# aleksandrina-streltsova/lidar-global-registration

Measured on AMD Instinct MI355X. Metric: scan-pair registrations/sec, higher is better.
Workload: dtype f32

## Files before the change

### lidar-global-registration_amd/csrc/lgr_match_sweep.cuh

```cuda
#pragma once
#include "lgr_match_common.cuh"
#include "lgr_match_mfma.cuh"

namespace {

constexpr int SW_RB = 1;
constexpr int SW_OCC = SW_RB == 1 ? 6 : 4;

__global__ void ucol_pack_kernel(const float* __restrict__ u_colv, int mb_pad, float c_scale, unsigned short* __restrict__ out) {
    const int col = blockIdx.x * blockDim.x + threadIdx.x;
    if (col >= mb_pad) return;
    const float t = ((fmaxf(u_colv[col], 0.f) * 1.00001f) * 1.0001f) * c_scale;
    const unsigned bits = t >= 0.f ? __float_as_uint(t) : 0x7f800000u;
    out[col] = (unsigned short) (min(bits + 0xffffu, 0x7f800000u) >> 16);
}

__global__ void pass_select_kernel(const unsigned long long* __restrict__ pass_stages, double half_of_all, const int* __restrict__ xcd_start ,
                                   int* __restrict__ xs_sweep, int* __restrict__ xs_plain) {
    const int i = threadIdx.x;
    if (i >= 9) return;
    const bool plain = pass_stages && (double) pass_stages[0] > half_of_all;
    xs_sweep[i] = plain ? 0 : xcd_start[i];
    xs_plain[i] = plain ? xcd_start[i] : 0;
}

__global__ __launch_bounds__(NTHR, SW_OCC) void match_sweep(const f16x8* __restrict__ Ap, const f16x8* __restrict__ Bp, size_t bset_stride ,
                                                            float c_scale, const int* __restrict__ blkcl, int ma_pad, int mb_pad, int rg_rows,
                                                            const unsigned* __restrict__ stage_mask, int n_cc, int item_rb, const int2* __restrict__ items,
                                                            const int* __restrict__ xcd_start, int* __restrict__ xcd_ctr, CoarseArgs ca,
                                                            const unsigned short* __restrict__ ucol16 ,
                                                            uint2* __restrict__ kept_out, unsigned long long* __restrict__ kept_count , unsigned kept_cap) {
    typedef f16x8 frag;
    constexpr int NF = OpFmt<FMT_F16R>::NF;
    constexpr int STAGE_FRAGS = STAGE_TILES * NF * 64;
    constexpr int CO_FRAGS = STAGE_TILES * 2 * 64, CO_NB = 6, CO_D = 4;
    static_assert(CO_D == 4 && CO_NB == CO_D + 2, "the counted waits below are written for two pairs of stages in flight");
    static_assert(WAVES == 2 * STAGE_TILES, "one coarse piece per wave");
    __shared__ __attribute__((aligned(16))) unsigned char smem[CO_NB * CO_FRAGS * (int) sizeof(frag) + 16];
    int& item_s = *reinterpret_cast<int*>(smem + CO_NB * CO_FRAGS * (int) sizeof(frag));
    unsigned n_tested = 0u, n_rejected = 0u, n_skipped = 0u;
    const int xcd = blockIdx.x % 8;
    const int item0 = xcd_start[xcd], n_items = xcd_start[xcd + 1] - item0;
    const int tid = threadIdx.x, lane = tid & 63, wave = tid >> 6, half = lane >> 5;
    const int rg_blocks = rg_rows / BLOCK_ROWS;
    const int n_rb_total = ma_pad / BLOCK_ROWS;
    constexpr int IINF = 0x7f800000;
    const f32x16 nav = {0.f, 0.f, 0.f, 0.f, 0.f, 0.f, 0.f, 0.f, 0.f, 0.f, 0.f, 0.f, 0.f, 0.f, 0.f, 0.f};

    for (;;) {
        __syncthreads();
        if (tid == 0) item_s = n_items > 0 ? atomicAdd(&xcd_ctr[xcd], 1) : 0x7fffffff;
        __syncthreads();
        const int it = item_s;
        if (it >= n_items) break;
        const int2 item = items[item0 + it];
        const int cc = item.x, rb0 = item.y;
        const int n_rb = min(item_rb, n_rb_total - rb0);
        const int col_tile0 = cc * (CHUNK_COLS / TILE);
        const int n_coltiles = min(CHUNK_COLS / TILE, mb_pad / TILE - col_tile0);
        const int n_stages = n_coltiles / STAGE_TILES;
        const unsigned full = n_stages >= 32 ? 0xffffffffu : ((1u << n_stages) - 1u);
        unsigned my_mask = lane < n_rb ? (stage_mask[(size_t) (rb0 + lane) * n_cc + cc] & full) : 0u;

        for (int rbi = 0; rbi < n_rb;) {
            const int rbA = rb0 + rbi;
            const bool pair = SW_RB == 2 && rbi + 1 < n_rb && blkcl[rbA + 1] == blkcl[rbA];
            const unsigned mk[2] = {(unsigned) __builtin_amdgcn_readlane(my_mask, rbi), pair ? (unsigned) __builtin_amdgcn_readlane(my_mask, min(rbi + 1, 63)) : 0u};
            rbi += pair ? 2 : 1;
            const unsigned mask = mk[0] | mk[1];
            if (!mask) continue;
            const int set = blkcl[rbA];
            const frag* Bset = Bp + (size_t) set * bset_stride + (size_t) col_tile0 * NF * 64;
            int row_tile[2];
            frag a0[2], a1[2];
            int t_lane[2][2];
            float e_lane[2][2];
            float trow[2];
            unsigned long long skipm[2][2];
            unsigned kept[2][STAGE_TILES];
            const unsigned skipped_before = n_skipped;
#pragma unroll
            for (int r = 0; r < SW_RB; ++r) {
                row_tile[r] = (rbA + r) * (BLOCK_ROWS / TILE) + wave;
                const int rt = mk[r] ? row_tile[r] : row_tile[0];
                a0[r] = Ap[((size_t) rt * NF + 0) * 64 + lane];
                a1[r] = Ap[((size_t) rt * NF + 1) * 64 + lane];
                t_lane[r][0] = t_lane[r][1] = IINF; e_lane[r][0] = e_lane[r][1] = 0.f; trow[r] = 0.f;
                skipm[r][0] = skipm[r][1] = 0ull;
#pragma unroll
                for (int ct = 0; ct < STAGE_TILES; ++ct) kept[r][ct] = 0u;
            }
            asm volatile("s_waitcnt lgkmcnt(0)\n\ts_barrier" : : : "memory");
            unsigned to_issue = mask, to_do = mask;
            int issued = 0, done_ = 0;
            auto dma_coarse = [&]() {
                const int s_ = __builtin_ctz(to_issue);
                to_issue &= to_issue - 1u;
                const char* src = reinterpret_cast<const char*>(Bset + (size_t) s_ * STAGE_FRAGS + (size_t) ((wave >> 1) * NF + (wave & 1)) * 64);
                char* dst = reinterpret_cast<char*>(smem) + (issued % CO_NB) * (CO_FRAGS * (int) sizeof(frag)) + wave * 1024;
#ifndef LGR_EXP_SWEEP_NODMA
                __builtin_amdgcn_global_load_lds((const void*) (src + lane * 16), (__attribute__((address_space(3))) void*) dst, 16, 0, 0);
#else
                (void) src; (void) dst;
#endif
                ++issued;
            };
            while (issued < CO_D && to_issue) dma_coarse();
#pragma unroll
            for (int r = 0; r < SW_RB; ++r) {
                if (!mk[r]) continue;
                const int rb = rbA + r;
                const float ur = ca.u_rt[rb * (BLOCK_ROWS / TILE) + wave];
                if (ca.u_row) trow[r] = ((fmaxf(ca.u_row[(size_t) row_tile[r] * TILE + (lane & 31)], 0.f) * 1.00001f) * 1.0001f) * c_scale;
                const float x = ca.xmax[rb / rg_blocks];
#pragma unroll
                for (int h2 = 0; h2 < 2; ++h2) {
                    if (!(h2 ? (mk[r] >> 16) : (mk[r] & 0xffffu))) continue;
                    const int q = lane + 64 * h2;
                    const int gst = min(cc * STAGES_PER_CHUNK + (q >> 2), ca.n_stage_total - 1);
                    const int gct = min(col_tile0 + q, ca.n_ct_total - 1);
                    const float us = ca.u_stage ? __uint_as_float(ca.u_ct[gct]) : 0.f;
                    float xt = x, yt = ca.ymax[(size_t) set * ca.n_stage_total + gst];
                    if (ca.rt_shell) {
                        const float2 sa = ca.rt_shell[rb * (BLOCK_ROWS / TILE) + wave];
                        const float2 sb = ca.ct_shell[(size_t) set * ca.n_ct_total + gct];
                        const float gap = fmaxf(sb.x - sa.y, sa.x - sb.y) - 4e-6f * (sa.y + sb.y);
                        const float U = fmaxf(fmaxf(ur, us), 0.f);
                        const bool skip = gap > 0.f && gap * gap * (0.99999f * 0.99999f * 0.99999f) > U * 1.00001f + 1e-12f;
                        skipm[r][h2] = __ballot(skip);
                        xt = fminf(xt, sa.y); yt = fminf(yt, sb.y);
                    }
                    const float s = xt + yt;
                    const float et = (ca.quad * s) * s + ca.cross * (xt * yt) + ca.lin * s + ca.abs;
                    float t = fmaxf(fmaxf(ca.u_row ? 0.f : ur, us), 0.f) * 1.00001f + et;
                    t = (t * 1.0001f) * c_scale;
                    t_lane[r][h2] = t >= 0.f ? __float_as_int(t) : IINF;
                    e_lane[r][h2] = (et * 1.0001f) * c_scale;
                }
            }
            asm volatile("" : : "v"(t_lane[0][0]), "v"(t_lane[0][1]), "v"(e_lane[0][0]), "v"(e_lane[0][1]), "v"(trow[0]) : "memory");
            if (SW_RB == 2) asm volatile("" : : "v"(t_lane[1][0]), "v"(t_lane[1][1]), "v"(e_lane[1][0]), "v"(e_lane[1][1]), "v"(trow[1]) : "memory");
            auto compute = [&](int st, int buf) {
                const frag* cs = reinterpret_cast<const frag*>(smem) + buf * CO_FRAGS + lane;
                unsigned need[2];
#pragma unroll
                for (int r = 0; r < SW_RB; ++r) {
                    const unsigned sk4 = (unsigned) ((st < 16 ? skipm[r][0] : skipm[r][1]) >> ((st * STAGE_TILES) & 63)) & 0xfu;
                    const bool on = (mk[r] >> st) & 1u;
                    if (on) n_skipped += (unsigned) __builtin_popcount(sk4);
                    need[r] = on ? (~sk4 & 0xfu) : 0u;
                }
                if (!(need[0] | (SW_RB == 2 ? need[1] : 0u))) return;
#pragma unroll
                for (int ct = 0; ct < STAGE_TILES; ++ct) {
                    if (!(((need[0] | (SW_RB == 2 ? need[1] : 0u)) >> ct) & 1u)) continue;
                    const int q = st * STAGE_TILES + ct;
                    const frag c0 = cs[ct * 128], c1 = cs[ct * 128 + 64];
#pragma unroll
                    for (int r = 0; r < SW_RB; ++r) {
                        if (!((need[r] >> ct) & 1u)) continue;
                        f32x16 acc = mfma_step(c0, a0[r], nav);
                        acc = mfma_step(c1, a1[r], acc);
                        auto ai = [&](int g) { return __float_as_int(acc[g]); };
                        const int m0 = min(min(ai(0), ai(1)), ai(2)), m1 = min(min(ai(3), ai(4)), ai(5)), m2 = min(min(ai(6), ai(7)), ai(8));
                        const int m3 = min(min(ai(9), ai(10)), ai(11)), m4 = min(min(ai(12), ai(13)), ai(14));
                        const int m = min(min(min(m0, m1), m2), min(min(m3, m4), ai(15)));
                        const int t_sel = st < 16 ? t_lane[r][0] : t_lane[r][1];
                        const float e_sel = st < 16 ? e_lane[r][0] : e_lane[r][1];
                        const int tc = __builtin_amdgcn_readlane(t_sel, q & 63);
                        const float te = __uint_as_float(__builtin_amdgcn_readlane(__float_as_uint(e_sel), q & 63));
                        const int thr = max(__float_as_int(trow[r] + te), tc);
                        if (__ballot(m <= thr) == 0ull) continue;
                        bool kp = __ballot(m <= __float_as_int(trow[r] + te)) != 0ull;
                        if (!kp && ucol16) {
                            const unsigned short* uc = ucol16 + ((size_t) (col_tile0 + q) << 5) + 4 * half;
                            float dmin = 3.4028234663852886e38f;
#pragma unroll
                            for (int gq = 0; gq < 4; ++gq) {
                                const uint2 w = *reinterpret_cast<const uint2*>(uc + 8 * gq);
                                const float u0 = __uint_as_float(w.x << 16), u1 = __uint_as_float(w.x & 0xffff0000u);
                                const float u2 = __uint_as_float(w.y << 16), u3 = __uint_as_float(w.y & 0xffff0000u);
                                dmin = fminf(fminf(dmin, acc[4 * gq] - u0), acc[4 * gq + 1] - u1);
                                dmin = fminf(fminf(dmin, acc[4 * gq + 2] - u2), acc[4 * gq + 3] - u3);
                            }
                            kp = __ballot(dmin <= te) != 0ull;
                        } else if (!kp && !ucol16) kp = true;
                        if (kp) kept[r][ct] |= 1u << st;
                    }
                }
            };
            while (to_do) {
                const int st = __builtin_ctz(to_do);
                to_do &= to_do - 1u;
                int st2 = -1;
                if (to_do) { st2 = __builtin_ctz(to_do); to_do &= to_do - 1u; }
                const int n_now = st2 >= 0 ? 2 : 1;
                const int newer = issued - done_ - n_now;
                if (newer >= 2) asm volatile("s_waitcnt vmcnt(2)" : : : "memory");
                else if (newer == 1) asm volatile("s_waitcnt vmcnt(1)" : : : "memory");
                else asm volatile("s_waitcnt vmcnt(0)" : : : "memory");
                __builtin_amdgcn_s_barrier();
                if (to_issue) dma_coarse();
                if (to_issue) dma_coarse();
#ifndef LGR_EXP_SWEEP_NOCOMPUTE
                compute(st, done_ % CO_NB);
                if (st2 >= 0) compute(st2, (done_ + 1) % CO_NB);
#endif
                done_ += n_now;
            }
            unsigned nk = 0u;
#pragma unroll
            for (int r = 0; r < SW_RB; ++r)
#pragma unroll
                for (int ct = 0; ct < STAGE_TILES; ++ct) nk += (unsigned) __builtin_popcount(kept[r][ct]);
            {
                const unsigned swept = (unsigned) (STAGE_TILES * (__builtin_popcount(mk[0]) + (SW_RB == 2 ? __builtin_popcount(mk[1]) : 0))), sk_now = n_skipped - skipped_before;
                n_tested += swept - sk_now;
                n_rejected += swept - sk_now - nk;
            }
            if (nk) {
                unsigned long long base = 0ull;
                if (lane == 0) base = atomicAdd(kept_count, (unsigned long long) nk);
                base = ((unsigned long long) (unsigned) __builtin_amdgcn_readfirstlane((int) (base >> 32)) << 32) | (unsigned) __builtin_amdgcn_readfirstlane((int) (unsigned) base);
                unsigned off = 0u;
#pragma unroll
                for (int r = 0; r < SW_RB; ++r)
#pragma unroll
                    for (int ct = 0; ct < STAGE_TILES; ++ct) {
                        const unsigned m = kept[r][ct];
                        if (lane < 32 && ((m >> lane) & 1u)) {
                            const unsigned long long pos = base + off + (unsigned) __builtin_popcount(m & ((1u << lane) - 1u));
                            if (pos < (unsigned long long) kept_cap) kept_out[pos] = make_uint2((unsigned) row_tile[r], (unsigned) (col_tile0 + lane * STAGE_TILES + ct));
                        }
                        off += (unsigned) __builtin_popcount(m);
                    }
            }
        }
    }
    if (ca.cnt && lane == 0) {
        if (n_tested) atomicAdd(&ca.cnt[0], (unsigned long long) n_tested);
        if (n_rejected) atomicAdd(&ca.cnt[1], (unsigned long long) n_rejected);
        if (n_skipped) atomicAdd(&ca.cnt[2], (unsigned long long) n_skipped);
    }
}

__global__ void touched_kernel(const uint2* __restrict__ kept, const unsigned long long* __restrict__ kept_count, unsigned kept_cap, const int* __restrict__ xs_plain ,
                               const uint8_t* __restrict__ sched, const int* __restrict__ tile_leaf, int n_leaves, size_t n_pairs, uint8_t* __restrict__ touched ) {
    const size_t i0 = (size_t) blockIdx.x * blockDim.x + threadIdx.x, step = (size_t) gridDim.x * blockDim.x;
    if (xs_plain[8] > 0 || *kept_count > (unsigned long long) kept_cap) {
        for (size_t i = i0; i < n_pairs; i += step) touched[i] = sched[i];
        return;
    }
    const size_t n = (size_t) *kept_count;
    for (size_t e = i0; e < n; e += step) {
        const uint2 ent = kept[e];
        const size_t idx = (size_t) (ent.x / (BLOCK_ROWS / TILE)) * n_leaves + tile_leaf[ent.y];
        touched[idx] = sched[idx];
    }
}

constexpr int TL_WAVES = 4, TL_RUN = 4;
template <bool COLDIR>
__global__ __launch_bounds__(64 * TL_WAVES) void match_tiles(const f16x8* __restrict__ Ap, const f16x8* __restrict__ Bp, size_t bset_stride, float out_scale,
                                                             const int* __restrict__ blkcl, int ma_pad, int mb_pad, int rg_rows, const int* __restrict__ tile_group,
                                                             int* __restrict__ rowmin, int* __restrict__ colmin, const uint2* __restrict__ kept,
                                                             const unsigned long long* __restrict__ kept_count, unsigned kept_cap) {
    typedef f16x8 frag;
    constexpr int NF = OpFmt<FMT_F16R>::NF;
    constexpr int IINF = 0x7f800000;
    const int lane = threadIdx.x & 63, half = lane >> 5;
    if (*kept_count > (unsigned long long) kept_cap) return;
    const unsigned n = (unsigned) *kept_count;
    const unsigned n_waves = gridDim.x * TL_WAVES, w_id = blockIdx.x * TL_WAVES + (threadIdx.x >> 6);
    const int rg_blocks = rg_rows / BLOCK_ROWS;
    const f32x16 nav = {0.f, 0.f, 0.f, 0.f, 0.f, 0.f, 0.f, 0.f, 0.f, 0.f, 0.f, 0.f, 0.f, 0.f, 0.f, 0.f};
    frag a[NF];
    unsigned cur_rt = 0xffffffffu;
    for (unsigned e0 = w_id * TL_RUN; e0 < n; e0 += n_waves * TL_RUN) {
        for (unsigned e = e0; e < min(n, e0 + TL_RUN); ++e) {
            const uint2 ent = kept[e];
            const unsigned rt = ent.x, ct = ent.y;
            const int rb = (int) (rt / (BLOCK_ROWS / TILE));
            if (rt != cur_rt) {
                cur_rt = rt;
#pragma unroll
                for (int kk = 0; kk < NF; ++kk) a[kk] = Ap[((size_t) rt * NF + kk) * 64 + lane];
            }
            const frag* bsrc = Bp + (size_t) blkcl[rb] * bset_stride + (size_t) ct * NF * 64 + lane;
            frag b[NF];
#pragma unroll
            for (int kk = 0; kk < NF; ++kk) b[kk] = bsrc[kk * 64];
            const f32x16 acc = mfma_chain<FMT_F16R>(a, b, nav);
            if (COLDIR) {
                int cm = min(__float_as_int(acc[0]), __float_as_int(acc[1]));
#pragma unroll
                for (int g = 2; g < 16; g += 2) cm = min(min(cm, __float_as_int(acc[g])), __float_as_int(acc[g + 1]));
                cm = min(cm, __shfl_xor(cm, 32));
                if (lane < 32 && cm != IINF) {
                    const int v = __float_as_int(__int_as_float(cm) * out_scale);
                    atomicMin(&colmin[(size_t) (rb / rg_blocks) * mb_pad + (size_t) ct * TILE + lane], v);
                }
            }
            {
                int rmin[16];
#pragma unroll
                for (int g = 0; g < 16; ++g) rmin[g] = __float_as_int(acc[g]);
                int w8[8], w4[4], w2[2], w1;
#pragma unroll
                for (int j = 0; j < 8; ++j) {
                    auto sw = __builtin_amdgcn_permlane16_swap((unsigned) rmin[j], (unsigned) rmin[8 + j], false, false);
                    w8[j] = min((int) sw[0], (int) sw[1]);
                }
                {
                    const bool up = (lane & 8) != 0;
#pragma unroll
                    for (int j = 0; j < 4; ++j) {
                        int keep = up ? w8[4 + j] : w8[j], send = up ? w8[j] : w8[4 + j];
                        w4[j] = min(keep, __builtin_amdgcn_update_dpp(0, send, 0x128 , 0xf, 0xf, true));
                    }
                }
                {
                    const bool up = (lane & 4) != 0;
#pragma unroll
                    for (int j = 0; j < 2; ++j) {
                        int keep = up ? w4[2 + j] : w4[j], send = up ? w4[j] : w4[2 + j];
                        const int t = __builtin_amdgcn_update_dpp(0, send, 0x141 , 0xf, 0xf, true);
                        w2[j] = min(keep, __builtin_amdgcn_update_dpp(0, t, 0x1b , 0xf, 0xf, true));
                    }
                }
                {
                    const bool up = (lane & 2) != 0;
                    int keep = up ? w2[1] : w2[0], send = up ? w2[0] : w2[1];
                    w1 = min(keep, __builtin_amdgcn_update_dpp(0, send, 0x4e , 0xf, 0xf, true));
                }
                w1 = min(w1, __builtin_amdgcn_update_dpp(0, w1, 0xb1 , 0xf, 0xf, true));
                const int g = (lane >> 1) & 15;
                w1 = __float_as_int(__int_as_float(w1) * out_scale);
                if ((lane & 1) == 0 && w1 != IINF)
                    atomicMin(&rowmin[(size_t) tile_group[ct] * ma_pad + (size_t) rt * TILE + (g & 3) + 8 * (g >> 2) + 4 * half], w1);
            }
        }
    }
}

}
```

Measured before the change: 45.94.

## Restructure sweep inner loop around tile walker with lane-indexed kept masks

Removes the unused two-row-block path and rewrites the match_sweep stage loop through a new iterator header. Stage pairs are walked as 8-tile intervals with precomputed need masks, and half-crossing state (thresholds, skip masks) is switched in place. Kept tiles are now recorded as 64-bit lane-indexed masks and written out with mbcnt instead of per-tile popcounts. It also makes wave uniform via readfirstlane and adds an optional, off-by-default LDS lookahead prefetch. The intent is fewer registers, less scalar/vector bookkeeping and a simpler output scatter, at the cost of a more intricate iteration helper that must stay consistent with the ring layout.

```diff
diff --git a/lidar-global-registration_amd/csrc/lgr_match_sweep.cuh b/lidar-global-registration_amd/csrc/lgr_match_sweep.cuh
--- a/lidar-global-registration_amd/csrc/lgr_match_sweep.cuh
+++ b/lidar-global-registration_amd/csrc/lgr_match_sweep.cuh
@@ -1,11 +1,16 @@
 #pragma once
 #include "lgr_match_common.cuh"
 #include "lgr_match_mfma.cuh"
+#include "lgr_sweep_iter.h"
 
 namespace {
 
-constexpr int SW_RB = 1;
-constexpr int SW_OCC = SW_RB == 1 ? 6 : 4;
+constexpr int SW_OCC = 6;
+#ifdef LGR_EXP_SWEEP_LOOKAHEAD
+constexpr bool SW_LOOKAHEAD = true;
+#else
+constexpr bool SW_LOOKAHEAD = false;
+#endif
 
 __global__ void ucol_pack_kernel(const float* __restrict__ u_colv, int mb_pad, float c_scale, unsigned short* __restrict__ out) {
     const int col = blockIdx.x * blockDim.x + threadIdx.x;
@@ -33,15 +38,20 @@
     typedef f16x8 frag;
     constexpr int NF = OpFmt<FMT_F16R>::NF;
     constexpr int STAGE_FRAGS = STAGE_TILES * NF * 64;
-    constexpr int CO_FRAGS = STAGE_TILES * 2 * 64, CO_NB = 6, CO_D = 4;
+    constexpr int CO_FRAGS = STAGE_TILES * 2 * 64, CO_NB = SW_RING, CO_D = 4;
+    constexpr int SLOT_BYTES = CO_FRAGS * (int) sizeof(frag), TILE_BYTES = SLOT_BYTES / STAGE_TILES;
     static_assert(CO_D == 4 && CO_NB == CO_D + 2, "the counted waits below are written for two pairs of stages in flight");
     static_assert(WAVES == 2 * STAGE_TILES, "one coarse piece per wave");
-    __shared__ __attribute__((aligned(16))) unsigned char smem[CO_NB * CO_FRAGS * (int) sizeof(frag) + 16];
-    int& item_s = *reinterpret_cast<int*>(smem + CO_NB * CO_FRAGS * (int) sizeof(frag));
+    static_assert(STAGE_TILES == SW_STAGE_TILES && STAGES_PER_CHUNK == 2 * SW_HALF_STAGES, "lgr_sweep_iter.h walks this layout");
+    __shared__ __attribute__((aligned(16))) unsigned char smem[CO_NB * SLOT_BYTES + 16];
+    int& item_s = *reinterpret_cast<int*>(smem + CO_NB * SLOT_BYTES);
     unsigned n_tested = 0u, n_rejected = 0u, n_skipped = 0u;
     const int xcd = blockIdx.x % 8;
     const int item0 = xcd_start[xcd], n_items = xcd_start[xcd + 1] - item0;
-    const int tid = threadIdx.x, lane = tid & 63, wave = tid >> 6, half = lane >> 5;
+    const int tid = threadIdx.x, lane = tid & 63;
+    const int wave = __builtin_amdgcn_readfirstlane(tid >> 6);
+    const unsigned lane16 = (unsigned) lane * 16u;
+    auto lane_off = [&]() { unsigned v = lane16; asm volatile("" : "+v"(v)); return v; };
     const int rg_blocks = rg_rows / BLOCK_ROWS;
     const int n_rb_total = ma_pad / BLOCK_ROWS;
     constexpr int IINF = 0x7f800000;
@@ -62,159 +72,142 @@
         const unsigned full = n_stages >= 32 ? 0xffffffffu : ((1u << n_stages) - 1u);
         unsigned my_mask = lane < n_rb ? (stage_mask[(size_t) (rb0 + lane) * n_cc + cc] & full) : 0u;
 
-        for (int rbi = 0; rbi < n_rb;) {
-            const int rbA = rb0 + rbi;
-            const bool pair = SW_RB == 2 && rbi + 1 < n_rb && blkcl[rbA + 1] == blkcl[rbA];
-            const unsigned mk[2] = {(unsigned) __builtin_amdgcn_readlane(my_mask, rbi), pair ? (unsigned) __builtin_amdgcn_readlane(my_mask, min(rbi + 1, 63)) : 0u};
-            rbi += pair ? 2 : 1;
-            const unsigned mask = mk[0] | mk[1];
+        for (int rbi = 0; rbi < n_rb; ++rbi) {
+            const int rb = rb0 + rbi;
+            const unsigned mask = (unsigned) __builtin_amdgcn_readlane(my_mask, rbi);
             if (!mask) continue;
-            const int set = blkcl[rbA];
-            const frag* Bset = Bp + (size_t) set * bset_stride + (size_t) col_tile0 * NF * 64;
-            int row_tile[2];
-            frag a0[2], a1[2];
-            int t_lane[2][2];
-            float e_lane[2][2];
-            float trow[2];
-            unsigned long long skipm[2][2];
-            unsigned kept[2][STAGE_TILES];
-            const unsigned skipped_before = n_skipped;
-#pragma unroll
-            for (int r = 0; r < SW_RB; ++r) {
-                row_tile[r] = (rbA + r) * (BLOCK_ROWS / TILE) + wave;
-                const int rt = mk[r] ? row_tile[r] : row_tile[0];
-                a0[r] = Ap[((size_t) rt * NF + 0) * 64 + lane];
-                a1[r] = Ap[((size_t) rt * NF + 1) * 64 + lane];
-                t_lane[r][0] = t_lane[r][1] = IINF; e_lane[r][0] = e_lane[r][1] = 0.f; trow[r] = 0.f;
-                skipm[r][0] = skipm[r][1] = 0ull;
-#pragma unroll
-                for (int ct = 0; ct < STAGE_TILES; ++ct) kept[r][ct] = 0u;
-            }
+            const int set = blkcl[rb];
+            const char* const Bwave = reinterpret_cast<const char*>(Bp + (size_t) set * bset_stride + (size_t) col_tile0 * NF * 64 + (size_t) ((wave >> 1) * NF + (wave & 1)) * 64);
+            const int row_tile = rb * (BLOCK_ROWS / TILE) + wave;
+            const frag* const Arow = Ap + (size_t) row_tile * NF * 64;
+            const unsigned a_off = lane_off();
+            const frag a0 = *reinterpret_cast<const frag*>(reinterpret_cast<const char*>(Arow) + a_off);
+            const frag a1 = *reinterpret_cast<const frag*>(reinterpret_cast<const char*>(Arow + 64) + a_off);
+            int t_lane[2] = {IINF, IINF};
+            float e_lane[2] = {0.f, 0.f};
+            float trow = 0.f;
+            unsigned long long skipm[2] = {0ull, 0ull};
             asm volatile("s_waitcnt lgkmcnt(0)\n\ts_barrier" : : : "memory");
-            unsigned to_issue = mask, to_do = mask;
-            int issued = 0, done_ = 0;
+            unsigned to_issue = mask;
+            int islot = 0;
             auto dma_coarse = [&]() {
                 const int s_ = __builtin_ctz(to_issue);
                 to_issue &= to_issue - 1u;
-                const char* src = reinterpret_cast<const char*>(Bset + (size_t) s_ * STAGE_FRAGS + (size_t) ((wave >> 1) * NF + (wave & 1)) * 64);
-                char* dst = reinterpret_cast<char*>(smem) + (issued % CO_NB) * (CO_FRAGS * (int) sizeof(frag)) + wave * 1024;
+                const char* src = Bwave + (size_t) s_ * (STAGE_FRAGS * sizeof(frag));
+                char* dst = reinterpret_cast<char*>(smem) + islot * SLOT_BYTES + wave * 1024;
 #ifndef LGR_EXP_SWEEP_NODMA
-                __builtin_amdgcn_global_load_lds((const void*) (src + lane * 16), (__attribute__((address_space(3))) void*) dst, 16, 0, 0);
+                __builtin_amdgcn_global_load_lds((const void*) (src + lane_off()), (__attribute__((address_space(3))) void*) dst, 16, 0, 0);
 #else
                 (void) src; (void) dst;
 #endif
-                ++issued;
+                islot = sw_ring_next(islot);
             };
-            while (issued < CO_D && to_issue) dma_coarse();
-#pragma unroll
-            for (int r = 0; r < SW_RB; ++r) {
-                if (!mk[r]) continue;
-                const int rb = rbA + r;
-                const float ur = ca.u_rt[rb * (BLOCK_ROWS / TILE) + wave];
-                if (ca.u_row) trow[r] = ((fmaxf(ca.u_row[(size_t) row_tile[r] * TILE + (lane & 31)], 0.f) * 1.00001f) * 1.0001f) * c_scale;
+#pragma unroll
+            for (int i = 0; i < CO_D; ++i)
+                if (to_issue) dma_coarse();
+            {
+                const float ur = ca.u_rt[row_tile];
+                if (ca.u_row) trow = ((fmaxf(ca.u_row[(size_t) row_tile * TILE + (lane & 31)], 0.f) * 1.00001f) * 1.0001f) * c_scale;
                 const float x = ca.xmax[rb / rg_blocks];
 #pragma unroll
                 for (int h2 = 0; h2 < 2; ++h2) {
-                    if (!(h2 ? (mk[r] >> 16) : (mk[r] & 0xffffu))) continue;
+                    if (!(h2 ? (mask >> 16) : (mask & 0xffffu))) continue;
                     const int q = lane + 64 * h2;
                     const int gst = min(cc * STAGES_PER_CHUNK + (q >> 2), ca.n_stage_total - 1);
                     const int gct = min(col_tile0 + q, ca.n_ct_total - 1);
                     const float us = ca.u_stage ? __uint_as_float(ca.u_ct[gct]) : 0.f;
                     float xt = x, yt = ca.ymax[(size_t) set * ca.n_stage_total + gst];
                     if (ca.rt_shell) {
-                        const float2 sa = ca.rt_shell[rb * (BLOCK_ROWS / TILE) + wave];
+                        const float2 sa = ca.rt_shell[row_tile];
                         const float2 sb = ca.ct_shell[(size_t) set * ca.n_ct_total + gct];
                         const float gap = fmaxf(sb.x - sa.y, sa.x - sb.y) - 4e-6f * (sa.y + sb.y);
                         const float U = fmaxf(fmaxf(ur, us), 0.f);
                         const bool skip = gap > 0.f && gap * gap * (0.99999f * 0.99999f * 0.99999f) > U * 1.00001f + 1e-12f;
-                        skipm[r][h2] = __ballot(skip);
+                        skipm[h2] = __ballot(skip);
                         xt = fminf(xt, sa.y); yt = fminf(yt, sb.y);
                     }
                     const float s = xt + yt;
                     const float et = (ca.quad * s) * s + ca.cross * (xt * yt) + ca.lin * s + ca.abs;
                     float t = fmaxf(fmaxf(ca.u_row ? 0.f : ur, us), 0.f) * 1.00001f + et;
                     t = (t * 1.0001f) * c_scale;
-                    t_lane[r][h2] = t >= 0.f ? __float_as_int(t) : IINF;
-                    e_lane[r][h2] = (et * 1.0001f) * c_scale;
-                }
-            }
-            asm volatile("" : : "v"(t_lane[0][0]), "v"(t_lane[0][1]), "v"(e_lane[0][0]), "v"(e_lane[0][1]), "v"(trow[0]) : "memory");
-            if (SW_RB == 2) asm volatile("" : : "v"(t_lane[1][0]), "v"(t_lane[1][1]), "v"(e_lane[1][0]), "v"(e_lane[1][1]), "v"(trow[1]) : "memory");
-            auto compute = [&](int st, int buf) {
-                const frag* cs = reinterpret_cast<const frag*>(smem) + buf * CO_FRAGS + lane;
-                unsigned need[2];
-#pragma unroll
-                for (int r = 0; r < SW_RB; ++r) {
-                    const unsigned sk4 = (unsigned) ((st < 16 ? skipm[r][0] : skipm[r][1]) >> ((st * STAGE_TILES) & 63)) & 0xfu;
-                    const bool on = (mk[r] >> st) & 1u;
-                    if (on) n_skipped += (unsigned) __builtin_popcount(sk4);
-                    need[r] = on ? (~sk4 & 0xfu) : 0u;
-                }
-                if (!(need[0] | (SW_RB == 2 ? need[1] : 0u))) return;
-#pragma unroll
-                for (int ct = 0; ct < STAGE_TILES; ++ct) {
-                    if (!(((need[0] | (SW_RB == 2 ? need[1] : 0u)) >> ct) & 1u)) continue;
-                    const int q = st * STAGE_TILES + ct;
-                    const frag c0 = cs[ct * 128], c1 = cs[ct * 128 + 64];
-#pragma unroll
-                    for (int r = 0; r < SW_RB; ++r) {
-                        if (!((need[r] >> ct) & 1u)) continue;
-                        f32x16 acc = mfma_step(c0, a0[r], nav);
-                        acc = mfma_step(c1, a1[r], acc);
-                        auto ai = [&](int g) { return __float_as_int(acc[g]); };
-                        const int m0 = min(min(ai(0), ai(1)), ai(2)), m1 = min(min(ai(3), ai(4)), ai(5)), m2 = min(min(ai(6), ai(7)), ai(8));
-                        const int m3 = min(min(ai(9), ai(10)), ai(11)), m4 = min(min(ai(12), ai(13)), ai(14));
-                        const int m = min(min(min(m0, m1), m2), min(min(m3, m4), ai(15)));
-                        const int t_sel = st < 16 ? t_lane[r][0] : t_lane[r][1];
-                        const float e_sel = st < 16 ? e_lane[r][0] : e_lane[r][1];
-                        const int tc = __builtin_amdgcn_readlane(t_sel, q & 63);
-                        const float te = __uint_as_float(__builtin_amdgcn_readlane(__float_as_uint(e_sel), q & 63));
-                        const int thr = max(__float_as_int(trow[r] + te), tc);
-                        if (__ballot(m <= thr) == 0ull) continue;
-                        bool kp = __ballot(m <= __float_as_int(trow[r] + te)) != 0ull;
-                        if (!kp && ucol16) {
-                            const unsigned short* uc = ucol16 + ((size_t) (col_tile0 + q) << 5) + 4 * half;
-                            float dmin = 3.4028234663852886e38f;
-#pragma unroll
-                            for (int gq = 0; gq < 4; ++gq) {
-                                const uint2 w = *reinterpret_cast<const uint2*>(uc + 8 * gq);
-                                const float u0 = __uint_as_float(w.x << 16), u1 = __uint_as_float(w.x & 0xffff0000u);
-                                const float u2 = __uint_as_float(w.y << 16), u3 = __uint_as_float(w.y & 0xffff0000u);
-                                dmin = fminf(fminf(dmin, acc[4 * gq] - u0), acc[4 * gq + 1] - u1);
-                                dmin = fminf(fminf(dmin, acc[4 * gq + 2] - u2), acc[4 * gq + 3] - u3);
-                            }
-                            kp = __ballot(dmin <= te) != 0ull;
-                        } else if (!kp && !ucol16) kp = true;
-                        if (kp) kept[r][ct] |= 1u << st;
+                    t_lane[h2] = t >= 0.f ? __float_as_int(t) : IINF;
+                    e_lane[h2] = (et * 1.0001f) * c_scale;
+                }
+            }
+            asm volatile("" : : "v"(t_lane[0]), "v"(t_lane[1]), "v"(e_lane[0]), "v"(e_lane[1]), "v"(trow) : "memory");
+            __builtin_amdgcn_s_waitcnt(0x0070);
+            int half_end = SW_HALF_STAGES, q_half = 0;
+            int t_cur = t_lane[0];
+            float e_cur = e_lane[0];
+            unsigned long long kept_lo = 0ull, kept_cur = 0ull;
+            const frag* const ring = reinterpret_cast<const frag*>(smem + lane16);
+            frag c0, c1;
+            f32x16 acc;
+            auto ring_request = [&](int tile) {
+                const frag* p = reinterpret_cast<const frag*>(reinterpret_cast<const char*>(ring) + tile * TILE_BYTES);
+                c0 = p[0]; c1 = p[64];
+            };
+            auto tile_start = [&]() {
+                acc = mfma_step(c0, a0, nav);
+                acc = mfma_step(c1, a1, acc);
+            };
+            auto tile_finish = [&](int lane_q) {
+                auto ai = [&](int g) { return __float_as_int(acc[g]); };
+                const int m0 = min(min(ai(0), ai(1)), ai(2)), m1 = min(min(ai(3), ai(4)), ai(5)), m2 = min(min(ai(6), ai(7)), ai(8));
+                const int m3 = min(min(ai(9), ai(10)), ai(11)), m4 = min(min(ai(12), ai(13)), ai(14));
+                const int m = min(min(min(m0, m1), m2), min(min(m3, m4), ai(15)));
+                const int tc = __builtin_amdgcn_readlane(t_cur, lane_q);
+                const float te = __uint_as_float(__builtin_amdgcn_readlane(__float_as_uint(e_cur), lane_q));
+                const int thr = max(__float_as_int(trow + te), tc);
+                if (__ballot(m <= thr) == 0ull) return;
+                bool kp = __ballot(m <= __float_as_int(trow + te)) != 0ull;
+                if (!kp && ucol16) {
+                    const unsigned short* uc = ucol16 + ((size_t) (col_tile0 + q_half + lane_q) << 5) + (lane_off() >> 9) * 4u;
+                    float dmin = 3.4028234663852886e38f;
+#pragma unroll
+                    for (int gq = 0; gq < 4; ++gq) {
+                        const uint2 w = *reinterpret_cast<const uint2*>(uc + 8 * gq);
+                        const float u0 = __uint_as_float(w.x << 16), u1 = __uint_as_float(w.x & 0xffff0000u);
+                        const float u2 = __uint_as_float(w.y << 16), u3 = __uint_as_float(w.y & 0xffff0000u);
+                        dmin = fminf(fminf(dmin, acc[4 * gq] - u0), acc[4 * gq + 1] - u1);
+                        dmin = fminf(fminf(dmin, acc[4 * gq + 2] - u2), acc[4 * gq + 3] - u3);
                     }
-                }
+                    kp = __ballot(dmin <= te) != 0ull;
+                } else if (!kp && !ucol16) kp = true;
+                if (kp) kept_cur |= 1ull << lane_q;
             };
+            unsigned long long skip_cur = skipm[0];
+            auto to_upper = [&]() { half_end = 2 * SW_HALF_STAGES; q_half = 64; skip_cur = skipm[1]; t_cur = t_lane[1]; e_cur = e_lane[1]; kept_lo = kept_cur; kept_cur = 0ull; };
+            unsigned to_do = mask;
+            int cslot = 0;
             while (to_do) {
-                const int st = __builtin_ctz(to_do);
-                to_do &= to_do - 1u;
-                int st2 = -1;
-                if (to_do) { st2 = __builtin_ctz(to_do); to_do &= to_do - 1u; }
-                const int n_now = st2 >= 0 ? 2 : 1;
-                const int newer = issued - done_ - n_now;
+                const SwInterval iv = sw_next_interval(to_do);
+                to_do = iv.rest;
+                const SwCrossing cross = sw_crossing(half_end, iv);
+                if (cross.first) to_upper();
+                const unsigned need8 = sw_need8(skip_cur, skipm[1], iv, cross.mid);
+                const int newer = sw_newer_requests(iv.rest);
                 if (newer >= 2) asm volatile("s_waitcnt vmcnt(2)" : : : "memory");
                 else if (newer == 1) asm volatile("s_waitcnt vmcnt(1)" : : : "memory");
                 else asm volatile("s_waitcnt vmcnt(0)" : : : "memory");
                 __builtin_amdgcn_s_barrier();
+#ifndef LGR_EXP_SWEEP_NOCOMPUTE
+                if (SW_LOOKAHEAD && need8) ring_request(sw_first_tile(need8, cslot));
+#endif
                 if (to_issue) dma_coarse();
                 if (to_issue) dma_coarse();
 #ifndef LGR_EXP_SWEEP_NOCOMPUTE
-                compute(st, done_ % CO_NB);
-                if (st2 >= 0) compute(st2, (done_ + 1) % CO_NB);
+                sw_walk8<SW_LOOKAHEAD>(need8, cslot, iv, cross.mid, ring_request, tile_start, tile_finish, to_upper);
 #endif
-                done_ += n_now;
-            }
-            unsigned nk = 0u;
-#pragma unroll
-            for (int r = 0; r < SW_RB; ++r)
-#pragma unroll
-                for (int ct = 0; ct < STAGE_TILES; ++ct) nk += (unsigned) __builtin_popcount(kept[r][ct]);
+                cslot = sw_ring_next2(cslot);
+            }
+            const unsigned long long kept_hi = q_half ? kept_cur : 0ull;
+            if (!q_half) kept_lo = kept_cur;
+            const unsigned nk_lo = (unsigned) __builtin_popcountll(kept_lo), nk = nk_lo + (unsigned) __builtin_popcountll(kept_hi);
             {
-                const unsigned swept = (unsigned) (STAGE_TILES * (__builtin_popcount(mk[0]) + (SW_RB == 2 ? __builtin_popcount(mk[1]) : 0))), sk_now = n_skipped - skipped_before;
+                unsigned swept, sk_now;
+                sw_visit_counts(mask, skipm[0], skipm[1], swept, sk_now);
+                n_skipped += sk_now;
                 n_tested += swept - sk_now;
                 n_rejected += swept - sk_now - nk;
             }
@@ -222,18 +215,15 @@
                 unsigned long long base = 0ull;
                 if (lane == 0) base = atomicAdd(kept_count, (unsigned long long) nk);
                 base = ((unsigned long long) (unsigned) __builtin_amdgcn_readfirstlane((int) (base >> 32)) << 32) | (unsigned) __builtin_amdgcn_readfirstlane((int) (unsigned) base);
-                unsigned off = 0u;
-#pragma unroll
-                for (int r = 0; r < SW_RB; ++r)
-#pragma unroll
-                    for (int ct = 0; ct < STAGE_TILES; ++ct) {
-                        const unsigned m = kept[r][ct];
-                        if (lane < 32 && ((m >> lane) & 1u)) {
-                            const unsigned long long pos = base + off + (unsigned) __builtin_popcount(m & ((1u << lane) - 1u));
-                            if (pos < (unsigned long long) kept_cap) kept_out[pos] = make_uint2((unsigned) row_tile[r], (unsigned) (col_tile0 + lane * STAGE_TILES + ct));
-                        }
-                        off += (unsigned) __builtin_popcount(m);
-                    }
+                auto n_below = [&](unsigned long long m) { return __builtin_amdgcn_mbcnt_hi((unsigned) (m >> 32), __builtin_amdgcn_mbcnt_lo((unsigned) m, 0u)); };
+                if ((kept_lo >> lane) & 1ull) {
+                    const unsigned long long pos = base + n_below(kept_lo);
+                    if (pos < (unsigned long long) kept_cap) kept_out[pos] = make_uint2((unsigned) row_tile, (unsigned) (col_tile0 + lane));
+                }
+                if ((kept_hi >> lane) & 1ull) {
+                    const unsigned long long pos = base + nk_lo + n_below(kept_hi);
+                    if (pos < (unsigned long long) kept_cap) kept_out[pos] = make_uint2((unsigned) row_tile, (unsigned) (col_tile0 + 64 + lane));
+                }
             }
         }
     }
diff --git a/lidar-global-registration_amd/csrc/lgr_sweep_iter.h b/lidar-global-registration_amd/csrc/lgr_sweep_iter.h
--- /dev/null
+++ b/lidar-global-registration_amd/csrc/lgr_sweep_iter.h
@@ -0,0 +1,74 @@
+#pragma once
+
+#if defined(__HIPCC__)
+#define LGR_SWEEP_FN __host__ __device__ __forceinline__
+#else
+#define LGR_SWEEP_FN inline
+#endif
+
+constexpr int SW_STAGE_TILES = 4;
+constexpr int SW_RING = 6;
+constexpr int SW_HALF_STAGES = 16;
+static_assert(SW_RING % 2 == 0, "an interval's two stages lie in neighbouring slots only when the ring never wraps inside a pair");
+
+LGR_SWEEP_FN unsigned sw_need4(unsigned long long skip_lo, unsigned long long skip_hi, int st) {
+    const unsigned long long w = st < SW_HALF_STAGES ? skip_lo : skip_hi;
+    return ~(unsigned) (w >> ((st * SW_STAGE_TILES) & 63)) & 0xfu;
+}
+
+struct SwInterval { int st, st2; unsigned rest; };
+LGR_SWEEP_FN SwInterval sw_next_interval(unsigned to_do ) {
+    SwInterval iv;
+    iv.st = __builtin_ctz(to_do);
+    to_do &= to_do - 1u;
+    iv.st2 = -1;
+    if (to_do) { iv.st2 = __builtin_ctz(to_do); to_do &= to_do - 1u; }
+    iv.rest = to_do;
+    return iv;
+}
+LGR_SWEEP_FN unsigned sw_need8(unsigned long long skip_cur, unsigned long long skip_hi, SwInterval iv, bool mid) {
+    unsigned n = ~(unsigned) (skip_cur >> ((iv.st * SW_STAGE_TILES) & 63)) & 0xfu;
+    if (iv.st2 >= 0) n |= (~(unsigned) ((mid ? skip_hi : skip_cur) >> ((iv.st2 * SW_STAGE_TILES) & 63)) & 0xfu) << SW_STAGE_TILES;
+    return n;
+}
+struct SwCrossing { bool first, mid; };
+LGR_SWEEP_FN SwCrossing sw_crossing(int half_end, SwInterval iv) {
+    SwCrossing c = {iv.st >= half_end, false};
+    c.mid = !c.first && iv.st2 >= half_end;
+    return c;
+}
+LGR_SWEEP_FN int sw_newer_requests(unsigned rest) { return rest == 0u ? 0 : ((rest & (rest - 1u)) == 0u ? 1 : 2); }
+LGR_SWEEP_FN int sw_ring_next(int slot) { return slot == SW_RING - 1 ? 0 : slot + 1; }
+LGR_SWEEP_FN int sw_ring_next2(int slot ) { return slot == SW_RING - 2 ? 0 : slot + 2; }
+
+LGR_SWEEP_FN int sw_first_tile(unsigned need8 , int slot ) { return slot * SW_STAGE_TILES + __builtin_ctz(need8); }
+template <bool LOOKAHEAD = true, class Request, class Start, class Finish, class ToUpper>
+LGR_SWEEP_FN void sw_walk8(unsigned need8, int slot , SwInterval iv, bool mid, Request&& request, Start&& start, Finish&& finish, ToUpper&& to_upper) {
+    need8 &= 0xffu;
+    const int qa = (iv.st * SW_STAGE_TILES) & 63, qb = (iv.st2 * SW_STAGE_TILES) & 63;
+#if defined(__HIPCC__)
+#pragma unroll
+#endif
+    for (int b = 0; b < 2 * SW_STAGE_TILES; ++b) {
+        if (b == SW_STAGE_TILES && mid) to_upper();
+        if (!((need8 >> b) & 1u)) continue;
+        if (!LOOKAHEAD) request(slot * SW_STAGE_TILES + b);
+        start();
+        const unsigned rem = need8 >> (b + 1);
+        if (LOOKAHEAD && rem) request(slot * SW_STAGE_TILES + b + 1 + __builtin_ctz(rem));
+        finish((b < SW_STAGE_TILES ? qa : qb) | (b & (SW_STAGE_TILES - 1)));
+    }
+}
+
+LGR_SWEEP_FN unsigned long long sw_expand4(unsigned m16) {
+    unsigned long long x = m16 & 0xffffu;
+    x = (x | (x << 24)) & 0x000000ff000000ffull;
+    x = (x | (x << 12)) & 0x000f000f000f000full;
+    x = (x | (x << 6)) & 0x0303030303030303ull;
+    x = (x | (x << 3)) & 0x1111111111111111ull;
+    return x * 15ull;
+}
+LGR_SWEEP_FN void sw_visit_counts(unsigned mask, unsigned long long skip_lo, unsigned long long skip_hi, unsigned& swept, unsigned& skipped) {
+    swept = (unsigned) (SW_STAGE_TILES * __builtin_popcount(mask));
+    skipped = (unsigned) (__builtin_popcountll(sw_expand4(mask & 0xffffu) & skip_lo) + __builtin_popcountll(sw_expand4(mask >> 16) & skip_hi));
+}
```

Result: no change. 45.90 (-0.1%).
